# teasgen/speech_separation

Hardware: NVIDIA B200
Metric: dptn_av_separated_audio_seconds_per_second (higher is better)
Workload: dtype f16

## Files before the change

include/vatss.h:

```cpp
#ifndef VATSS_H_
#define VATSS_H_

#include <stddef.h>
#include <stdint.h>

#ifdef __cplusplus
extern "C" {
#endif

#define VATSS_ABI_VERSION 1

#define VATSS_KIND_DPTN_AV 0
#define VATSS_KIND_DPTN_WAV 1
#define VATSS_KIND_DPTN_MASK 2
#define VATSS_KIND_DPRNN 3

#define VATSS_ENGINE_AUTO 0
#define VATSS_ENGINE_GENERIC 1
#define VATSS_ENGINE_TENSOR 2
#define VATSS_ENGINE_TENSOR_F16RES 3

typedef struct vatss_model_desc {
  int32_t kind;
  int32_t N;
// ... 80 lines not shown
                    double* summary_out, double* scratch, void* stream);

int vatss_pit_sisdr(const float* s1p, const float* s2p, const float* s1, const float* s2, const float* mix, int B,
                    int T, int zero_mean, double* rows_out, double* summary_out, double* scratch, void* stream);

size_t vatss_sdr_workspace_bytes(int B, int T, int filter_length);
int vatss_sdr(const float* s1p, const float* s2p, const float* s1, const float* s2, const float* mix, int B, int T,
              int filter_length, int zero_mean, double load_diag, double* rows_out, double* summary_out,
              void* workspace, size_t workspace_bytes, void* stream);

int vatss_pit_sisnr_backward(const float* s1p, const float* s2p, const float* s1, const float* s2, int B, int T,
                             const double* scratch, const double* summary, const float* grad_out, float* grad_s1p,
                             float* grad_s2p, void* stream);

int vatss_tc_gemm(int epi, const void* A16, long long lda, const void* W16, const float* bias, const float* res,
                  long long ldr, const float* ln_w, const float* ln_b, float* out32, long long ldo32, void* out16,
                  long long ldo16, int act16, const float* prelu_a, long long M, int NOUT, int K, void* stream);

int vatss_tc_gemm_ln16(const void* A16, long long lda, const void* W16, const float* bias, const void* res16,
                       long long ldr16, const float* ln_w, const float* ln_b, float* out32, long long ldo32,
                       void* out16, long long ldo16, int act16, const float* prelu_a, long long M, int NOUT, int K,
                       void* stream);

int vatss_tc_lstm(const void* x16, const void* x16lo ,
                  const float* const* lstm_params ,
                  void* out16, int mode, int B, int S, int C, int N, int ndir, int act, void* wpack,
                  float* bias_pack, void* stream);

int vatss_tc_attention(const void* qkv16, void* out16, int mode, int B, int S, int C, int N, int heads, int force_simt,
                       void* stream);

int vatss_generic_gemm(const float* A, long long lda, const float* W, const float* bias, const float* bias2,
                       const float* R, long long ldr, float* out, long long ldc, long long M, int NOUT, int K, int act,
                       const float* prelu_a, void* stream);
int vatss_generic_layernorm(const float* in, const float* res, const float* w, const float* b, float* out,
                            long long rows, int N, int mode, void* stream);
int vatss_generic_attention(const float* qkv, float* out, int mode, int B, int S, int C, int N, int heads,
                            void* stream);
int vatss_generic_lstm(const float* pre, const float* whh_f, const float* whh_r, float* out, int mode, int B, int S,
                       int C, int H, int ndir, void* stream);

int vatss_tc_tail(const vatss_model_desc* d, const float* const* params, int n_params, const void* packed,
                  const void* x16, const float* enc, int B, int T, float* s1_pred, float* s2_pred,
                  void* workspace, size_t workspace_bytes, void* stream);

int vatss_longform_windows(int T, int W, int H);
int vatss_window_cut(const float* mix, const float* emb1, const float* emb2, int R, int T, int Tv, int E, int W, int H,
                     int spf, int first, int count, float* mix_out, float* emb1_out, float* emb2_out, void* stream);
size_t vatss_window_stitch_scratch_bytes(int R, int n);
int vatss_window_stitch(const float* y1, const float* y2, int R, int T, int W, int H, float* s1, float* s2,
                        uint8_t* swaps_out, double* corr_out, void* scratch, size_t scratch_bytes, void* stream);

size_t vatss_stoi_workspace_bytes(int B, int T, int fs);
int vatss_stoi(const float* s1p, const float* s2p, const float* s1, const float* s2, int B, int T, int fs, int extended,
               double* rows_out, int* kept_out, double* summary_out, void* workspace, size_t workspace_bytes,
               void* stream);

#define VATSS_STAGE_COUNT 9
unsigned long long vatss_launch_count(void);
void vatss_debug_lstm_trace(void* dev_buffer);
void vatss_debug_cta_limit(int ctas);
void vatss_debug_lstm_pingpong(int on);
void vatss_debug_lstm_groups(int groups);
void vatss_debug_tail_staged(int on);
void vatss_debug_gemm_l2_order(int on);
void vatss_debug_attention_version(int v);
int vatss_profile_begin(void);
int vatss_profile_end(float* ms_per_stage, int* launches_per_stage, int n_stages);

#define VATSS_LIP_NCONV 25
#define VATSS_LIP_PSLOTS 6
#define VATSS_LIP_ENGINE_F32 0
#define VATSS_LIP_ENGINE_TENSOR 1
void vatss_debug_lipreader(int flags);
void vatss_debug_lipreader_kernel(int version);
void vatss_debug_lipreader_trace(void* dev_buffer);
#define VATSS_LIP_NSTAGES 26
void vatss_debug_lipreader_capture(void* const* stages, int n);
size_t vatss_lipreader_packed_bytes(void);
size_t vatss_lipreader_workspace_bytes(int B, int T, int Hc, int Wc);
int vatss_lipreader_pack_weights(const float* const* params, int n_params, int relu_type, void* packed,
                                 size_t packed_bytes, void* stream);
int vatss_lipreader_forward(const void* packed, size_t packed_bytes, int relu_type, const float* video, int B, int T,
                            int Hin, int Win, int y0, int x0, int Hc, int Wc, float pre_scale, float pre_shift,
                            float* out, void* workspace, size_t workspace_bytes, int engine, void* stream);

#ifdef __cplusplus
}
#endif
// ... 2 lines not shown
```

speech_separation_b200/_lib.py:

```python
import ctypes
import os

_HERE = os.path.dirname(os.path.abspath(__file__))
LIB_PATH = os.environ.get("VATSS_LIB_OVERRIDE") or os.path.join(_HERE, "libvatss_b200.so")

KIND = {"dptn_av": 0, "dptn_wav": 1, "dptn_mask": 2, "dprnn": 3}
ENGINE = {"auto": 0, "generic": 1, "tensor": 2, "tensor-f16res": 3}

P_GLOBAL = [
    "encoder.weight", "decoder.weight", "visual_compression.weight", "visual_compression.bias", "gate",
    "video_ln.weight", "video_ln.bias", "dprnn.speakers_separation.0.weight",
    "dprnn.speakers_separation.1.weight", "dprnn.speakers_separation.1.bias",
    "HEAD_W", "HEAD_B", "dprnn.output_gate.0.weight", "dprnn.output_gate.0.bias",
]
S_DPTN = [
    "mha.in_proj_weight", "mha.in_proj_bias", "mha.out_proj.weight", "mha.out_proj.bias", "ln1.weight", "ln1.bias",
    "rnn.weight_ih_l0", "rnn.weight_hh_l0", "rnn.bias_ih_l0", "rnn.bias_hh_l0",
    "rnn.weight_ih_l0_reverse", "rnn.weight_hh_l0_reverse", "rnn.bias_ih_l0_reverse", "rnn.bias_hh_l0_reverse",
    "ffn.1.weight", "ffn.1.bias", "ln2.weight", "ln2.bias",
]
S_DPRNN = [
    None, None, None, None, None, None,
    "rnn.weight_ih_l0", "rnn.weight_hh_l0", "rnn.bias_ih_l0", "rnn.bias_hh_l0",
    "rnn.weight_ih_l0_reverse", "rnn.weight_hh_l0_reverse", "rnn.bias_ih_l0_reverse", "rnn.bias_hh_l0_reverse",
# ... 16 lines not shown
    "vatss_pack_weights": (ctypes.c_int, [ctypes.POINTER(ModelDesc), ctypes.POINTER(ctypes.c_void_p), ctypes.c_int,
                                          ctypes.c_void_p, ctypes.c_size_t, ctypes.c_void_p]),
    "vatss_forward": (ctypes.c_int, [ctypes.POINTER(ModelDesc), ctypes.POINTER(ctypes.c_void_p), ctypes.c_int,
                                     ctypes.c_void_p, ctypes.c_void_p, ctypes.c_void_p, ctypes.c_void_p,
                                     ctypes.c_int, ctypes.c_int, ctypes.c_int, ctypes.c_void_p, ctypes.c_void_p,
                                     ctypes.c_void_p, ctypes.c_size_t, ctypes.c_void_p]),
    "vatss_segment": (ctypes.c_int, [ctypes.c_void_p] + [ctypes.c_int] * 5 + [ctypes.c_void_p, ctypes.c_void_p]),
    "vatss_overlap_add": (ctypes.c_int, [ctypes.c_void_p] + [ctypes.c_int] * 5 + [ctypes.c_void_p, ctypes.c_void_p]),
    "vatss_encoder": (ctypes.c_int, [ctypes.POINTER(ModelDesc), ctypes.POINTER(ctypes.c_void_p), ctypes.c_void_p,
                                     ctypes.c_void_p, ctypes.c_void_p, ctypes.c_int, ctypes.c_int, ctypes.c_int,
                                     ctypes.c_void_p, ctypes.c_void_p, ctypes.c_void_p, ctypes.c_void_p]),
    "vatss_decoder": (ctypes.c_int, [ctypes.POINTER(ModelDesc), ctypes.c_void_p, ctypes.c_void_p, ctypes.c_int,
                                     ctypes.c_int, ctypes.c_void_p, ctypes.c_void_p, ctypes.c_void_p]),
    "vatss_tc_gemm": (ctypes.c_int, [ctypes.c_int, ctypes.c_void_p, ctypes.c_longlong, ctypes.c_void_p, ctypes.c_void_p,
                                     ctypes.c_void_p, ctypes.c_longlong, ctypes.c_void_p, ctypes.c_void_p,
                                     ctypes.c_void_p, ctypes.c_longlong, ctypes.c_void_p, ctypes.c_longlong,
                                     ctypes.c_int, ctypes.c_void_p, ctypes.c_longlong, ctypes.c_int, ctypes.c_int,
                                     ctypes.c_void_p]),
    "vatss_tc_gemm_ln16": (ctypes.c_int, [ctypes.c_void_p, ctypes.c_longlong, ctypes.c_void_p, ctypes.c_void_p,
                                          ctypes.c_void_p, ctypes.c_longlong, ctypes.c_void_p, ctypes.c_void_p,
                                          ctypes.c_void_p, ctypes.c_longlong, ctypes.c_void_p, ctypes.c_longlong,
                                          ctypes.c_int, ctypes.c_void_p, ctypes.c_longlong, ctypes.c_int, ctypes.c_int,
                                          ctypes.c_void_p]),
    "vatss_tc_lstm": (ctypes.c_int, [ctypes.c_void_p, ctypes.c_void_p, ctypes.POINTER(ctypes.c_void_p), ctypes.c_void_p] +
                      [ctypes.c_int] * 7 + [ctypes.c_void_p, ctypes.c_void_p, ctypes.c_void_p]),
    "vatss_tc_attention": (ctypes.c_int, [ctypes.c_void_p, ctypes.c_void_p] + [ctypes.c_int] * 7 + [ctypes.c_void_p]),
    "vatss_generic_gemm": (ctypes.c_int, [ctypes.c_void_p, ctypes.c_longlong] + [ctypes.c_void_p] * 4 +
                           [ctypes.c_longlong, ctypes.c_void_p, ctypes.c_longlong, ctypes.c_longlong, ctypes.c_int,
                            ctypes.c_int, ctypes.c_int, ctypes.c_void_p, ctypes.c_void_p]),
    "vatss_generic_layernorm": (ctypes.c_int, [ctypes.c_void_p] * 5 + [ctypes.c_longlong, ctypes.c_int, ctypes.c_int,
                                                                       ctypes.c_void_p]),
    "vatss_generic_attention": (ctypes.c_int, [ctypes.c_void_p, ctypes.c_void_p] + [ctypes.c_int] * 6 +
                                [ctypes.c_void_p]),
    "vatss_generic_lstm": (ctypes.c_int, [ctypes.c_void_p] * 4 + [ctypes.c_int] * 6 + [ctypes.c_void_p]),
    "vatss_tc_tail": (ctypes.c_int,[ctypes.POINTER(ModelDesc), ctypes.POINTER(ctypes.c_void_p), ctypes.c_int,
                                     ctypes.c_void_p, ctypes.c_void_p, ctypes.c_void_p, ctypes.c_int, ctypes.c_int,
                                     ctypes.c_void_p, ctypes.c_void_p, ctypes.c_void_p, ctypes.c_size_t,
                                     ctypes.c_void_p]),
    "vatss_launch_count": (ctypes.c_ulonglong, []),
    "vatss_engine_fallback_reason": (ctypes.c_char_p, [ctypes.POINTER(ModelDesc)]),
    "vatss_debug_lstm_trace": (None, [ctypes.c_void_p]),
    "vatss_debug_cta_limit": (None, [ctypes.c_int]),
    "vatss_debug_lstm_pingpong": (None, [ctypes.c_int]),
    "vatss_debug_lstm_groups": (None, [ctypes.c_int]),
    "vatss_debug_tail_staged": (None, [ctypes.c_int]),
    "vatss_debug_gemm_l2_order": (None, [ctypes.c_int]),
    "vatss_debug_attention_version": (None, [ctypes.c_int]),
    "vatss_profile_begin": (ctypes.c_int, []),
    "vatss_profile_end": (ctypes.c_int, [ctypes.POINTER(ctypes.c_float), ctypes.POINTER(ctypes.c_int), ctypes.c_int]),
    "vatss_sisnr_chunks": (ctypes.c_int, [ctypes.c_int]),
    "vatss_pit_sisnr": (ctypes.c_int, [ctypes.c_void_p] * 5 + [ctypes.c_int, ctypes.c_int] + [ctypes.c_void_p] * 5),
    "vatss_pit_sisdr": (ctypes.c_int, [ctypes.c_void_p] * 5 + [ctypes.c_int] * 3 + [ctypes.c_void_p] * 4),
    "vatss_sdr_workspace_bytes": (ctypes.c_size_t, [ctypes.c_int] * 3),
    "vatss_sdr": (ctypes.c_int, [ctypes.c_void_p] * 5 + [ctypes.c_int] * 4 + [ctypes.c_double] + [ctypes.c_void_p] * 3 +
                  [ctypes.c_size_t, ctypes.c_void_p]),
    "vatss_pit_sisnr_backward": (ctypes.c_int, [ctypes.c_void_p] * 4 + [ctypes.c_int, ctypes.c_int] + [ctypes.c_void_p] * 6),
    "vatss_longform_windows": (ctypes.c_int, [ctypes.c_int] * 3),
    "vatss_window_cut": (ctypes.c_int, [ctypes.c_void_p] * 3 + [ctypes.c_int] * 9 + [ctypes.c_void_p] * 4),
    "vatss_window_stitch_scratch_bytes": (ctypes.c_size_t, [ctypes.c_int, ctypes.c_int]),
    "vatss_window_stitch": (ctypes.c_int, [ctypes.c_void_p, ctypes.c_void_p] + [ctypes.c_int] * 4 +
                            [ctypes.c_void_p] * 5 + [ctypes.c_size_t, ctypes.c_void_p]),
    "vatss_stoi_workspace_bytes": (ctypes.c_size_t, [ctypes.c_int] * 3),
    "vatss_stoi": (ctypes.c_int, [ctypes.c_void_p] * 4 + [ctypes.c_int] * 4 + [ctypes.c_void_p] * 4 +
                   [ctypes.c_size_t, ctypes.c_void_p]),
    "vatss_debug_lipreader": (None, [ctypes.c_int]),
    "vatss_debug_lipreader_kernel": (None, [ctypes.c_int]),
    "vatss_debug_lipreader_trace": (None, [ctypes.c_void_p]),
    "vatss_debug_lipreader_capture": (None, [ctypes.POINTER(ctypes.c_void_p), ctypes.c_int]),
    "vatss_lipreader_packed_bytes": (ctypes.c_size_t, []),
    "vatss_lipreader_workspace_bytes": (ctypes.c_size_t, [ctypes.c_int] * 4),
# ... 76 lines not shown
```

speech_separation_b200/csrc/api.cu:

```cuda
#include <stdarg.h>
#include <string.h>

#include <atomic>
#include <mutex>
#include <string>
#include <vector>

#include "common.cuh"
#include "tensor_engine.cuh"
#include "tc_kernels.cuh"
#include "lipreader.cuh"

namespace vatss {

static thread_local std::string g_err;

void set_error(const char* fmt, ...) {
  char buf[1024];
  va_list ap;
  va_start(ap, fmt);
  vsnprintf(buf, sizeof(buf), fmt, ap);
  va_end(ap);
  g_err = buf;
}
// ... 346 lines not shown
  VATSS_CHECK_ARG(B > 0 && T >= d->K, "decoder: bad shape");
  const int L = (T - d->K) / stride_of(d) + 1;
  return launch_decoder(u, dec_w, B, L, d->N, d->K, T, proj_scratch, wav, (cudaStream_t)stream);
}

int vatss_tc_gemm(int epi, const void* A16, long long lda, const void* W16, const float* bias, const float* res,
                  long long ldr, const float* ln_w, const float* ln_b, float* out32, long long ldo32, void* out16,
                  long long ldo16, int act16, const float* prelu_a, long long M, int NOUT, int K, void* stream) {
  VATSS_CHECK_ARG(A16 && W16 && M >= 0, "tc_gemm: NULL operand");
  return launch_tc_gemm(epi, (const __half*)A16, lda, (const __half*)W16, bias, res, ldr, ln_w, ln_b, out32, ldo32,
                        (__half*)out16, ldo16, act16, prelu_a, M, NOUT, K, (cudaStream_t)stream);
}

int vatss_tc_gemm_ln16(const void* A16, long long lda, const void* W16, const float* bias, const void* res16,
                       long long ldr16, const float* ln_w, const float* ln_b, float* out32, long long ldo32,
                       void* out16, long long ldo16, int act16, const float* prelu_a, long long M, int NOUT, int K,
                       void* stream) {
  VATSS_CHECK_ARG(A16 && W16 && res16 && M >= 0, "tc_gemm_ln16: NULL operand");
  return launch_tc_gemm(TC_EPI_LN, (const __half*)A16, lda, (const __half*)W16, bias, nullptr, 0, ln_w, ln_b, out32,
                        ldo32, (__half*)out16, ldo16, act16, prelu_a, M, NOUT, K, (cudaStream_t)stream, nullptr, 0,
                        (const __half*)res16, ldr16);
}

int vatss_tc_lstm(const void* x16, const void* x16lo, const float* const* lp, void* out16, int mode, int B, int S, int C,
                  int N, int ndir, int act, void* wpack, float* bias_pack, void* stream) {
  VATSS_CHECK_ARG(x16 && lp && out16 && wpack && bias_pack, "tc_lstm: NULL pointer");
  VATSS_CHECK_ARG(ndir == 1 || ndir == 2, "tc_lstm: ndir must be 1 or 2");
  cudaStream_t st = (cudaStream_t)stream;
  for (int dir = 0; dir < ndir; ++dir) {
    int rc = launch_pack_lstm(lp[4 * dir + 0], lp[4 * dir + 1], lp[4 * dir + 2], lp[4 * dir + 3], N, dir,
                              x16lo != nullptr, (__half*)wpack, bias_pack, st);
    if (rc) return rc;
  }
  return launch_tc_lstm((const __half*)x16, (const __half*)x16lo, (const __half*)wpack, bias_pack, (__half*)out16, mode,
                        B, S, C, N, ndir,
                        act, st);
}

int vatss_tc_attention(const void* qkv16, void* out16, int mode, int B, int S, int C, int N, int heads, int force_simt,
                       void* stream) {
  VATSS_CHECK_ARG(qkv16 && out16 && heads > 0, "tc_attention: bad argument");
  const SeqMap map = mode == 0 ? intra_map(B, S, C) : inter_map(B, S, C);
  return launch_attention_f16((const __half*)qkv16, (__half*)out16, map, mode, B, S, C, N, heads, force_simt,
                              (cudaStream_t)stream);
}

// ... 30 lines not shown

int vatss_tc_tail(const vatss_model_desc* d, const float* const* params, int n_params, const void* packed,
                  const void* x16, const float* enc, int B, int T, float* s1_pred, float* s2_pred, void* workspace,
                  size_t workspace_bytes, void* stream) {
  if (check_desc(d)) return -1;
  VATSS_CHECK_ARG(params != nullptr && n_params == n_params_of(d), "parameter table has %d entries, expected %d",
                  n_params, n_params_of(d));
  VATSS_CHECK_ARG(tensor_engine_selected(d), "tc_tail: the model does not run on the TENSOR engine");
  VATSS_CHECK_ARG(packed && x16 && enc && s1_pred && s2_pred && workspace, "tc_tail: NULL pointer");
  Geometry g;
  if (geometry(d, B, T, 0, &g)) return -1;
  const size_t need = vatss_workspace_bytes(d, B, T, 0);
  VATSS_CHECK_ARG(workspace_bytes >= need, "workspace too small: %zu bytes given, %zu needed", workspace_bytes, need);
  return tensor_engine_tail(d, params, packed, (const __half*)x16, enc, g.B, g.T, 0, g.L, g.S, s1_pred, s2_pred,
                            workspace, (cudaStream_t)stream);
}

void vatss_debug_lstm_trace(void* dev_buffer) { vatss::g_lstm_trace = (long long*)dev_buffer; }
void vatss_debug_cta_limit(int ctas) { vatss::g_cta_limit = ctas; }
void vatss_debug_lstm_pingpong(int on) { vatss::g_lstm_pingpong = on; }
void vatss_debug_lstm_groups(int groups) { vatss::g_lstm_groups = groups; }
void vatss_debug_tail_staged(int on) { vatss::g_tail_staged = on; }
void vatss_debug_gemm_l2_order(int on) { vatss::g_gemm_l2_order = on; }
void vatss_debug_attention_version(int v) { vatss::g_attention_version = v == 1 ? 1 : 3; }

unsigned long long vatss_launch_count(void) { return g_launches.load(); }

int vatss_profile_begin(void) {
  std::lock_guard<std::mutex> lk(g_prof_mu);
  for (auto& r : g_prof) { cudaEventDestroy(r.a); cudaEventDestroy(r.b); }
  g_prof.clear();
  for (int i = 0; i < ST_COUNT; ++i) g_open[i] = -1;
  g_prof_on = true;
  return 0;
}

int vatss_profile_end(float* ms_per_stage, int* launches_per_stage, int n_stages) {
  std::lock_guard<std::mutex> lk(g_prof_mu);
  g_prof_on = false;
  VATSS_CHECK_ARG(ms_per_stage && launches_per_stage && n_stages >= ST_COUNT, "profile_end: need %d slots", ST_COUNT);
  for (int i = 0; i < n_stages; ++i) { ms_per_stage[i] = 0.f; launches_per_stage[i] = 0; }
  int rc = 0;
  for (auto& r : g_prof) {
    float ms = 0.f;
    if (cudaEventSynchronize(r.b) != cudaSuccess || cudaEventElapsedTime(&ms, r.a, r.b) != cudaSuccess) rc = -2;
    ms_per_stage[r.stage] += ms;
// ... 124 lines not shown
```

speech_separation_b200/csrc/tc_gemm.cu:

```cuda
#include "common.cuh"
#include "ptx.cuh"
#include "tc_kernels.cuh"

namespace vatss {

using namespace ptx;

typedef CUresult (*PFN_encodeTiled)(CUtensorMap*, CUtensorMapDataType, cuuint32_t, void*, const cuuint64_t*,
                                    const cuuint64_t*, const cuuint32_t*, const cuuint32_t*, CUtensorMapInterleave,
                                    CUtensorMapSwizzle, CUtensorMapL2promotion, CUtensorMapFloatOOBfill);

static PFN_encodeTiled get_encode() {
  static PFN_encodeTiled fn = nullptr;
  if (!fn) {
    void* p = nullptr;
    cudaDriverEntryPointQueryResult q;
    if (cudaGetDriverEntryPoint("cuTensorMapEncodeTiled", &p, cudaEnableDefault, &q) == cudaSuccess &&
        q == cudaDriverEntryPointSuccess)
      fn = reinterpret_cast<PFN_encodeTiled>(p);
  }
  return fn;
}

static int make_tmap_any(CUtensorMap* out, CUtensorMapDataType dt, const void* base, int rank, const uint64_t* dims,
// ... 571 lines not shown
  }
#define TCG_CASE(N_, K_, E_) \
  if (NOUT == N_ && KDIM == K_ && epi == E_) return tc_gemm_launch<N_, K_, E_>(A, lda, W, a, st);
  TCG_CASE(384, 128, TC_EPI_F16)
  TCG_CASE(128, 128, TC_EPI_LN)
  TCG_CASE(128, 256, TC_EPI_LN)
  TCG_CASE(128, 256, TC_EPI_LN_POST)
  TCG_CASE(128, 128, TC_EPI_LN_POST)
  TCG_CASE(256, 128, TC_EPI_F32)
  TCG_CASE(128, 128, TC_EPI_F32)
  TCG_CASE(192, 64, TC_EPI_F16)
  TCG_CASE(64, 64, TC_EPI_LN)
  TCG_CASE(64, 256, TC_EPI_LN)
  TCG_CASE(64, 128, TC_EPI_LN)
  TCG_CASE(64, 256, TC_EPI_LN_POST)
  TCG_CASE(64, 128, TC_EPI_LN_POST)
  TCG_CASE(128, 64, TC_EPI_F32)
  TCG_CASE(64, 64, TC_EPI_F32)
#undef TCG_CASE
  set_error("tc_gemm: no tensor-core instantiation for NOUT=%d K=%d epilogue=%d", NOUT, KDIM, epi);
  return -1;
}

}
```

speech_separation_b200/csrc/tc_kernels.cuh:

```cuda
#pragma once
#include <cuda_fp16.h>
#include <cuda_runtime.h>

#include "common.cuh"

namespace vatss {

enum { TC_EPI_F16 = 0, TC_EPI_F32 = 1, TC_EPI_LN = 2, TC_EPI_LN_POST = 3 };

int num_sms();
int grid_cap();
extern int g_cta_limit;
extern int g_lstm_pingpong;
extern int g_lstm_groups;
extern int g_tail_staged;
extern int g_gemm_l2_order;
extern long long* g_lstm_trace;

int launch_tc_gemm(int epi, const __half* A, long long lda, const __half* W, const float* bias, const float* res,
                   long long ldr, const float* ln_w, const float* ln_b, float* out32, long long ldo32, __half* out16,
                   long long ldo16, int act16, const float* prelu_a, long long M, int NOUT, int KDIM, cudaStream_t st,
                   __half* out16lo = nullptr, int wsplit = 0, const __half* res16 = nullptr, long long ldr16 = 0,
                   int reverse = 0, const __half* res16lo = nullptr);

int launch_tc_lstm(const __half* x16, const __half* x16lo, const __half* Wpack, const float* bias_pack, __half* out16,
                   int mode, int B, int S, int C, int NFEAT, int ndir, int act, cudaStream_t st);
int launch_pack_lstm(const float* Wih, const float* Whh, const float* bih, const float* bhh, int N, int dir,
                     int precise, __half* Wpack, float* bias_pack, cudaStream_t st);

int launch_attention_f16(const __half* qkv, __half* out, SeqMap map, int mode, int B, int S, int C, int N, int heads,
                         int force_simt, cudaStream_t st);

int launch_attention_v3(const __half* qkv, __half* out, SeqMap map, int mode, int B, int S, int C, int N, int heads,
                        cudaStream_t st);
extern int g_attention_version;

}
```

speech_separation_b200/csrc/tensor_engine.cu:

```cuda
#include "tensor_engine.cuh"

#include "tc_kernels.cuh"

#include <cstdlib>

namespace vatss {

int g_gemm_l2_order = -1;
int g_x16split = -1;
static bool x16split_enabled() {
  if (g_x16split < 0) {
    const char* e = getenv("VATSS_X16SPLIT");
    g_x16split = e ? atoi(e) : 1;
  }
  return g_x16split != 0;
}

namespace {

inline const float* sub_param(const float* const* params, int blk, int path, int slot) {
  return params[VATSS_P_GLOBAL_COUNT + (2 * blk + path) * VATSS_S_COUNT + slot];
}

struct Bump {
  char* base;
  size_t off = 0;
  explicit Bump(void* p) : base(reinterpret_cast<char*>(p)) {}
  template <typename T>
  T* take(size_t count) {
    T* r = reinterpret_cast<T*>(base + off);
    off += ((count * sizeof(T) + 1023) / 1024) * 1024;
    return r;
  }
};

struct SubPacked {
  __half* win;
  float* bin;
// ... 160 lines not shown
  if (d->kind == VATSS_KIND_DPTN_MASK) {
    if ((rc = to_half(params[VATSS_P_HGATE_W], p.wgate, N, N, 0, 1.f, st))) return rc;
  } else if ((rc = launch_fold_head(params[VATSS_P_HEAD_W], params[VATSS_P_HEAD_B], params[VATSS_P_DECODER_W], N, d->K,
                                    p.wfold, p.wdT, p.cfold, st)) ||
             (rc = launch_fold_spk(p.wfold, params[VATSS_P_SPK_W], params[VATSS_P_SPK_B], N, d->K, p.w2, p.c2, st))) {
    return rc;
  }
  return 0;
}

int tensor_engine_forward(const vatss_model_desc* d, const float* const* params, const void* packed,
                          const float* mix, const float* emb1, const float* emb2, int B, int T, int Tv, int L,
                          int S, float* s1_pred, float* s2_pred, void* workspace, cudaStream_t st) {
  Packed p;
  carve_packed(d, const_cast<void*>(packed), &p);
  Work w;
  carve_work(d, B, Tv, L, S, workspace, &w);
  const int N = d->N, H = d->H, C = d->C;
  const long long tok = (long long)B * S * C;
  const bool dprnn = d->kind == VATSS_KIND_DPRNN, av = d->kind == VATSS_KIND_DPTN_AV;
  const bool f16res = d->engine == VATSS_ENGINE_TENSOR_F16RES && !dprnn && d->kind != VATSS_KIND_DPTN_MASK;
  const bool y16res = d->kind != VATSS_KIND_DPTN_MASK;
  const bool x16split = !dprnn && d->kind != VATSS_KIND_DPTN_MASK && !f16res && x16split_enabled();
  int rc;
  {
    StageScope sc(ST_FRONTEND, st);
    if (av) {
      VATSS_CHECK_ARG(emb1 && emb2 && Tv > 0, "DPTN-AV needs both lip-embedding streams (Tv=%d)", Tv);
      if ((rc = launch_visual_compress(emb1, emb2, params[VATSS_P_VIS_W], params[VATSS_P_VIS_B], B, d->E, Tv, N, w.vis,
                                       st)))
        return rc;
    }
    if ((rc = launch_encoder(mix, params[VATSS_P_ENCODER_W], av ? w.vis : nullptr, params[VATSS_P_GATE],
                             params[VATSS_P_VLN_W], params[VATSS_P_VLN_B], B, T, Tv, N, d->K, L, S, C, d->P, w.enc32,
                             (f16res || x16split) ? nullptr : w.xa32, w.xa16, st, (dprnn || x16split) ? w.xa16lo : nullptr)))
      return rc;
  }
  for (int blk = 0; blk < d->num_blocks; ++blk)
    for (int path = 0; path < 2; ++path) {
      const int ndir = (path == 0 || d->bidir) ? 2 : 1;
      const SubPacked& s = p.sub[2 * blk + path];
      auto sp = [&](int slot) { return sub_param(params, blk, path, slot); };
      const SeqMap map = path == 0 ? intra_map(B, S, C) : inter_map(B, S, C);
      const bool last = (blk == d->num_blocks - 1) && path == 1;
      if (dprnn) {
        {
          StageScope sc(ST_LSTM_RECURRENT, st);
          if ((rc = launch_tc_lstm(w.xa16, w.xa16lo, s.wlstm, s.blstm, w.rnn16, path, B, S, C, N, ndir, 0, st))) return rc;
        }
        StageScope sc(ST_FFN_LN, st);
        if ((rc = launch_tc_gemm(TC_EPI_LN_POST, w.rnn16, ndir * H, s.wffn, sp(VATSS_S_FFN_B), w.xa32, N,
                                 sp(VATSS_S_LN2_W), sp(VATSS_S_LN2_B), w.xb32, N, w.xb16, N, last ? 2 : 0,
                                 params[VATSS_P_PRELU], tok, N, ndir * H, st, last ? nullptr : w.xb16lo, 1)))
          return rc;
        float* t32 = w.xa32; w.xa32 = w.xb32; w.xb32 = t32;
        __half* t16 = w.xa16; w.xa16 = w.xb16; w.xb16 = t16;
        t16 = w.xa16lo; w.xa16lo = w.xb16lo; w.xb16lo = t16;
      } else {
        {
          StageScope sc(ST_QKV, st);
          if ((rc = launch_tc_gemm(TC_EPI_F16, w.xa16, N, s.win, s.bin, nullptr, 0, nullptr, nullptr, nullptr, 0,
                                   w.qkv16, 3 * N, 0, nullptr, tok, 3 * N, N, st, nullptr, 0, nullptr, 0, g_gemm_l2_order)))
            return rc;
        }
        {
          StageScope sc(ST_ATTENTION, st);
          if ((rc = launch_attention_f16(w.qkv16, w.att16, map, path, B, S, C, N, d->heads, 0, st))) return rc;
        }
        {
          StageScope sc(ST_OUTPROJ_LN, st);
          if ((rc = launch_tc_gemm(TC_EPI_LN, w.att16, N, s.wout, sp(VATSS_S_OUTPROJ_B),
                                   (f16res || x16split) ? nullptr : w.xa32, N, sp(VATSS_S_LN1_W), sp(VATSS_S_LN1_B),
                                   y16res ? nullptr : w.xb32, N, w.xb16, N, 0, nullptr, tok, N, N, st, nullptr, 0,
                                   (f16res || x16split) ? w.xa16 : nullptr, N, g_gemm_l2_order,
                                   x16split ? w.xa16lo : nullptr)))
            return rc;
        }
        {
          StageScope sc(ST_LSTM_RECURRENT, st);
          if ((rc = launch_tc_lstm(w.xb16, nullptr, s.wlstm, s.blstm, w.rnn16, path, B, S, C, N, ndir, 1, st))) return rc;
        }
        StageScope sc(ST_FFN_LN, st);
        if ((rc = launch_tc_gemm(TC_EPI_LN, w.rnn16, ndir * H, s.wffn, sp(VATSS_S_FFN_B), y16res ? nullptr : w.xb32, N,
                                 sp(VATSS_S_LN2_W), sp(VATSS_S_LN2_B), (f16res || x16split || last) ? nullptr : w.xa32, N,
                                 w.xa16, N, last ? 2 : 0, params[VATSS_P_PRELU], tok, N, ndir * H, st,
                                 (x16split && !last) ? w.xa16lo : nullptr, 0, y16res ? w.xb16 : nullptr, N)))
          return rc;
      }
    }
  return tensor_engine_tail(d, params, packed, w.xa16, w.enc32, B, T, Tv, L, S, s1_pred, s2_pred, workspace, st);
}

int tensor_engine_tail(const vatss_model_desc* d, const float* const* params, const void* packed, const __half* x16,
                       const float* enc32, int B, int T, int Tv, int L, int S, float* s1_pred, float* s2_pred,
                       void* workspace, cudaStream_t st) {
  Packed p;
  carve_packed(d, const_cast<void*>(packed), &p);
  Work w;
  carve_work(d, B, Tv, L, S, workspace, &w);
  const int N = d->N, C = d->C;
  const long long tok = (long long)B * S * C, fr = (long long)B * L;
  int rc;
  StageScope sc(ST_TAIL, st);
  float* preds[2] = {s1_pred, s2_pred};
  if (d->kind != VATSS_KIND_DPTN_MASK) {
    rc = launch_tail_fused(x16, enc32, p.w2, p.c2, p.wdT, p.cfold, B, S, C, d->P, L, N, d->K, w.proj, st);
// ... 32 lines not shown
```

Baseline: 4354.

## Fuse FFN+LayerNorm GEMM with next sublayer's QKV projection in one kernel

Adds a clustered tcgen05 kernel that computes the FFN GEMM with residual add and LayerNorm, writes the normalized hi/lo f16 activations, and then reuses that tile from shared memory as the A operand for the following sublayer's QKV projection. The tensor engine calls it by default (env-controlled) for every non-last sublayer and skips the separate QKV GEMM. This removes one launch per sublayer and avoids re-reading the activation from global memory for QKV. In exchange it keeps both weight sets resident in shared memory and adds a more complex warp-specialized pipeline with cross-CTA barriers.

```diff
diff --git a/include/vatss.h b/include/vatss.h
--- a/include/vatss.h
+++ b/include/vatss.h
@@ -126,6 +126,10 @@
                        void* out16, long long ldo16, int act16, const float* prelu_a, long long M, int NOUT, int K,
                        void* stream);
 
+int vatss_tc_ffn_qkv(const void* rnn16, int KF, const void* Wffn16, const float* bffn, const void* y16,
+                     const float* ln_w, const float* ln_b, void* x16, void* x16lo, const void* Wqkv16,
+                     const float* bqkv, void* qkv16, long long M, int N, int fused, void* stream);
+
 int vatss_tc_lstm(const void* x16, const void* x16lo ,
                   const float* const* lstm_params ,
                   void* out16, int mode, int B, int S, int C, int N, int ndir, int act, void* wpack,
@@ -169,6 +173,7 @@
 void vatss_debug_tail_staged(int on);
 void vatss_debug_gemm_l2_order(int on);
 void vatss_debug_attention_version(int v);
+void vatss_debug_ffn_qkv_fused(int on);
 int vatss_profile_begin(void);
 int vatss_profile_end(float* ms_per_stage, int* launches_per_stage, int n_stages);
 
diff --git a/speech_separation_b200/_lib.py b/speech_separation_b200/_lib.py
--- a/speech_separation_b200/_lib.py
+++ b/speech_separation_b200/_lib.py
@@ -62,6 +62,8 @@
                                           ctypes.c_void_p, ctypes.c_longlong, ctypes.c_void_p, ctypes.c_longlong,
                                           ctypes.c_int, ctypes.c_void_p, ctypes.c_longlong, ctypes.c_int, ctypes.c_int,
                                           ctypes.c_void_p]),
+    "vatss_tc_ffn_qkv": (ctypes.c_int, [ctypes.c_void_p, ctypes.c_int] + [ctypes.c_void_p] * 10 +
+                         [ctypes.c_longlong, ctypes.c_int, ctypes.c_int, ctypes.c_void_p]),
     "vatss_tc_lstm": (ctypes.c_int, [ctypes.c_void_p, ctypes.c_void_p, ctypes.POINTER(ctypes.c_void_p), ctypes.c_void_p] +
                       [ctypes.c_int] * 7 + [ctypes.c_void_p, ctypes.c_void_p, ctypes.c_void_p]),
     "vatss_tc_attention": (ctypes.c_int, [ctypes.c_void_p, ctypes.c_void_p] + [ctypes.c_int] * 7 + [ctypes.c_void_p]),
@@ -86,6 +88,7 @@
     "vatss_debug_tail_staged": (None, [ctypes.c_int]),
     "vatss_debug_gemm_l2_order": (None, [ctypes.c_int]),
     "vatss_debug_attention_version": (None, [ctypes.c_int]),
+    "vatss_debug_ffn_qkv_fused": (None, [ctypes.c_int]),
     "vatss_profile_begin": (ctypes.c_int, []),
     "vatss_profile_end": (ctypes.c_int, [ctypes.POINTER(ctypes.c_float), ctypes.POINTER(ctypes.c_int), ctypes.c_int]),
     "vatss_sisnr_chunks": (ctypes.c_int, [ctypes.c_int]),
diff --git a/speech_separation_b200/csrc/api.cu b/speech_separation_b200/csrc/api.cu
--- a/speech_separation_b200/csrc/api.cu
+++ b/speech_separation_b200/csrc/api.cu
@@ -392,6 +392,22 @@
                         (const __half*)res16, ldr16);
 }
 
+int vatss_tc_ffn_qkv(const void* rnn16, int KF, const void* Wffn16, const float* bffn, const void* y16,
+                     const float* ln_w, const float* ln_b, void* x16, void* x16lo, const void* Wqkv16,
+                     const float* bqkv, void* qkv16, long long M, int N, int fused, void* stream) {
+  VATSS_CHECK_ARG(M >= 0, "tc_ffn_qkv: negative row count");
+  cudaStream_t st = (cudaStream_t)stream;
+  if (fused)
+    return launch_tc_ffn_qkv((const __half*)rnn16, KF, (const __half*)Wffn16, bffn, (const __half*)y16, ln_w, ln_b,
+                             (__half*)x16, (__half*)x16lo, (const __half*)Wqkv16, bqkv, (__half*)qkv16, M, N, st);
+  int rc = launch_tc_gemm(TC_EPI_LN, (const __half*)rnn16, KF, (const __half*)Wffn16, bffn, nullptr, N, ln_w, ln_b,
+                          nullptr, N, (__half*)x16, N, 0, nullptr, M, N, KF, st, (__half*)x16lo, 0,
+                          (const __half*)y16, N);
+  if (rc) return rc;
+  return launch_tc_gemm(TC_EPI_F16, (const __half*)x16, N, (const __half*)Wqkv16, bqkv, nullptr, 0, nullptr, nullptr,
+                        nullptr, 0, (__half*)qkv16, 3 * N, 0, nullptr, M, 3 * N, N, st);
+}
+
 int vatss_tc_lstm(const void* x16, const void* x16lo, const float* const* lp, void* out16, int mode, int B, int S, int C,
                   int N, int ndir, int act, void* wpack, float* bias_pack, void* stream) {
   VATSS_CHECK_ARG(x16 && lp && out16 && wpack && bias_pack, "tc_lstm: NULL pointer");
@@ -468,6 +484,7 @@
 void vatss_debug_lstm_groups(int groups) { vatss::g_lstm_groups = groups; }
 void vatss_debug_tail_staged(int on) { vatss::g_tail_staged = on; }
 void vatss_debug_gemm_l2_order(int on) { vatss::g_gemm_l2_order = on; }
+void vatss_debug_ffn_qkv_fused(int on) { vatss::g_ffn_qkv_fused = on; }
 void vatss_debug_attention_version(int v) { vatss::g_attention_version = v == 1 ? 1 : 3; }
 
 unsigned long long vatss_launch_count(void) { return g_launches.load(); }
diff --git a/speech_separation_b200/csrc/tc_gemm.cu b/speech_separation_b200/csrc/tc_gemm.cu
--- a/speech_separation_b200/csrc/tc_gemm.cu
+++ b/speech_separation_b200/csrc/tc_gemm.cu
@@ -617,4 +617,398 @@
   return -1;
 }
 
-}
+template <int N, int KF>
+struct FfnQkvSmem {
+  static constexpr int KBF = KF / 64;
+  static constexpr int KBQ = N / 64;
+  static constexpr int WROW = (N / 2) * 128;
+  static constexpr int OFF_WF = 0;
+  static constexpr int OFF_WQ = OFF_WF + KBF * WROW;
+  static constexpr int OFF_A = OFF_WQ + 3 * KBQ * WROW;
+  static constexpr int OFF_Y = OFF_A + KBF * 16384;
+  static constexpr int OFF_PAR = OFF_Y + KBQ * 16384;
+  static constexpr int OFF_BAR = OFF_PAR + 6 * N * 4;
+  static constexpr int OFF_XCH = OFF_BAR + 256;
+  static constexpr int OFF_STAGE = OFF_XCH + 2048;
+  static constexpr int EPW = 8;
+  static constexpr int THREADS = 64 + 32 * EPW;
+  static constexpr int TOTAL = OFF_STAGE + EPW * 32 * STG_LD * 4 + 1024;
+  static constexpr int TMEM_COLS = 4 * N <= 256 ? 256 : 512;
+  static_assert(4 * N <= 512 && N % 64 == 0 && KF % 64 == 0, "shape");
+};
+
+struct FfnQkvArgs {
+  long long M;
+  int num_pairs;
+  const float* bffn;
+  const float* ln_w;
+  const float* ln_b;
+  const float* bqkv;
+  __half* x16;
+  __half* x16lo;
+  __half* qkv16;
+};
+
+template <int N, int KF>
+__global__ void __cluster_dims__(2, 1, 1) __launch_bounds__(FfnQkvSmem<N, KF>::THREADS, 1)
+k_tc_ffn_qkv(const __grid_constant__ CUtensorMap tmapA, const __grid_constant__ CUtensorMap tmapY,
+             const __grid_constant__ CUtensorMap tmapWf, const __grid_constant__ CUtensorMap tmapWq, FfnQkvArgs p) {
+  using L = FfnQkvSmem<N, KF>;
+  extern __shared__ unsigned char smem_raw[];
+  const uint32_t base = (smem_u32(smem_raw) + 1023u) & ~1023u;
+  unsigned char* gen = smem_raw + (base - smem_u32(smem_raw));
+  const uint32_t sWf = base + L::OFF_WF, sWq = base + L::OFF_WQ, sA = base + L::OFF_A, sY = base + L::OFF_Y;
+  float* sPar = reinterpret_cast<float*>(gen + L::OFF_PAR);
+  const uint32_t bars = base + L::OFF_BAR;
+  const uint32_t bar_w = bars;
+  const uint32_t bar_afull = bars + 8;
+  const uint32_t bar_aempty = bars + 16;
+  const uint32_t bar_yfull = bars + 24;
+  const uint32_t bar_yempty = bars + 32;
+  const uint32_t bar_ffull = bars + 40;
+  const uint32_t bar_fempty = bars + 56;
+  const uint32_t bar_xfull = bars + 72;
+  const uint32_t bar_qfull = bars + 80;
+  const uint32_t bar_qempty = bars + 96;
+  const uint32_t tmem_slot = bars + 128;
+
+  const int warp = threadIdx.x >> 5, lane = threadIdx.x & 31;
+  const uint32_t rank = cluster_ctarank();
+  const bool leader = rank == 0;
+  const int cluster = blockIdx.x >> 1, nclusters = gridDim.x >> 1;
+
+  if (threadIdx.x == 0) {
+    mbar_init(bar_w, 1);
+    mbar_init(bar_afull, 1);
+    mbar_init(bar_aempty, 1);
+    mbar_init(bar_yfull, 1);
+    mbar_init(bar_yempty, 1);
+    mbar_init(bar_xfull, 2 * L::EPW);
+    for (int s = 0; s < 2; ++s) {
+      mbar_init(bar_ffull + 8 * s, 1);
+      mbar_init(bar_fempty + 8 * s, 2 * L::EPW);
+      mbar_init(bar_qfull + 8 * s, 1);
+      mbar_init(bar_qempty + 8 * s, 2 * L::EPW);
+    }
+    fence_mbar_init();
+    prefetch_tmap(&tmapA);
+    prefetch_tmap(&tmapY);
+    prefetch_tmap(&tmapWf);
+    prefetch_tmap(&tmapWq);
+  }
+  for (int i = threadIdx.x; i < N; i += blockDim.x) {
+    sPar[i] = p.bffn[i];
+    sPar[N + i] = p.ln_w[i];
+    sPar[2 * N + i] = p.ln_b[i];
+  }
+  for (int i = threadIdx.x; i < 3 * N; i += blockDim.x) sPar[3 * N + i] = p.bqkv[i];
+  if (warp == 1) {
+    tmem_alloc<2>(tmem_slot, L::TMEM_COLS);
+    tmem_relinquish<2>();
+  }
+  tc_fence_before();
+  __syncthreads();
+  cluster_sync();
+  tc_fence_after();
+  const uint32_t tmem = *reinterpret_cast<volatile uint32_t*>(gen + L::OFF_BAR + 128);
+
+  if (threadIdx.x == 0) {
+    mbar_expect_tx(bar_w, (L::KBF + 3 * L::KBQ) * L::WROW);
+    for (int kb = 0; kb < L::KBF; ++kb) tma_load_2d(sWf + kb * L::WROW, &tmapWf, bar_w, kb * 64, (int)rank * (N / 2));
+    for (int ch = 0; ch < 3; ++ch)
+      for (int kb = 0; kb < L::KBQ; ++kb)
+        tma_load_2d(sWq + (ch * L::KBQ + kb) * L::WROW, &tmapWq, bar_w, kb * 64, ch * N + (int)rank * (N / 2));
+  }
+  mbar_wait(bar_w, 0);
+  cluster_sync();
+
+  if (warp == 0) {
+    if (lane == 0) {
+      uint32_t afull_leader;
+      asm volatile("mapa.shared::cluster.u32 %0, %1, 0;" : "=r"(afull_leader) : "r"(bar_afull));
+      int i = 0;
+      for (int pt = cluster; pt < p.num_pairs; pt += nclusters, ++i) {
+        const int row0 = pt * 256 + (int)rank * 128;
+        mbar_wait(bar_aempty, (i & 1) ^ 1);
+        if (leader) mbar_expect_tx(bar_afull, 2 * L::KBF * 16384);
+        for (int kb = 0; kb < L::KBF; ++kb) tma_load_2d_cg2(sA + kb * 16384, &tmapA, afull_leader, kb * 64, row0);
+        mbar_wait(bar_yempty, (i & 1) ^ 1);
+        mbar_expect_tx(bar_yfull, L::KBQ * 16384);
+        for (int cb = 0; cb < L::KBQ; ++cb) tma_load_2d(sY + cb * 16384, &tmapY, bar_yfull, cb * 64, row0);
+      }
+    }
+    __syncwarp();
+  } else if (warp == 1) {
+    if (leader && lane == 0) {
+      constexpr uint32_t IDESC = idesc_f16(256, N, 0);
+      int i = 0;
+      for (int pt = cluster; pt < p.num_pairs; pt += nclusters, ++i) {
+        const int fs = i & 1;
+        mbar_wait(bar_afull, i & 1);
+        mbar_wait(bar_fempty + 8 * fs, ((i >> 1) & 1) ^ 1);
+        tc_fence_after();
+#pragma unroll
+        for (int k16 = 0; k16 < KF / 16; ++k16) {
+          const int kb = k16 >> 2, kk = k16 & 3;
+          const uint64_t a = smem_desc_sw128_kmajor(sA + kb * 16384) + (uint64_t)(kk * 2);
+          const uint64_t b = smem_desc_sw128_kmajor(sWf + kb * L::WROW) + (uint64_t)(kk * 2);
+          umma_f16<2>(tmem + fs * N, a, b, IDESC, k16 > 0 ? 1u : 0u);
+        }
+        umma_commit_cg2(bar_aempty, 3);
+        umma_commit_cg2(bar_ffull + 8 * fs, 3);
+        mbar_wait(bar_xfull, i & 1);
+        tc_fence_after();
+#pragma unroll
+        for (int ch = 0; ch < 3; ++ch) {
+          const int j = i * 3 + ch, qs = j & 1;
+          mbar_wait(bar_qempty + 8 * qs, ((j >> 1) & 1) ^ 1);
+          tc_fence_after();
+#pragma unroll
+          for (int k16 = 0; k16 < N / 16; ++k16) {
+            const int kb = k16 >> 2, kk = k16 & 3;
+            const uint64_t a = smem_desc_sw128_kmajor(sY + kb * 16384) + (uint64_t)(kk * 2);
+            const uint64_t b = smem_desc_sw128_kmajor(sWq + (ch * L::KBQ + kb) * L::WROW) + (uint64_t)(kk * 2);
+            umma_f16<2>(tmem + 2 * N + qs * N, a, b, IDESC, k16 > 0 ? 1u : 0u);
+          }
+          if (ch == 2) umma_commit_cg2(bar_yempty, 3);
+          umma_commit_cg2(bar_qfull + 8 * qs, 3);
+        }
+      }
+    }
+    __syncwarp();
+  } else {
+    const int q = warp & 3, half = (warp - 2) >> 2;
+    constexpr int NC = N / 2;
+    const int cbase = half * NC;
+    const int rr = q * 32 + lane;
+    const float* sBias = sPar;
+    const float* sLw = sPar + N;
+    const float* sLb = sPar + 2 * N;
+    const float* sBq = sPar + 3 * N;
+    float* xch = reinterpret_cast<float*>(gen + L::OFF_XCH);
+    float* stage = reinterpret_cast<float*>(gen + L::OFF_STAGE) + (warp - 2) * 32 * STG_LD;
+    uint32_t fempty_leader[2], qempty_leader[2], xfull_leader;
+    for (int s = 0; s < 2; ++s) {
+      asm volatile("mapa.shared::cluster.u32 %0, %1, 0;" : "=r"(fempty_leader[s]) : "r"(bar_fempty + 8 * s));
+      asm volatile("mapa.shared::cluster.u32 %0, %1, 0;" : "=r"(qempty_leader[s]) : "r"(bar_qempty + 8 * s));
+    }
+    asm volatile("mapa.shared::cluster.u32 %0, %1, 0;" : "=r"(xfull_leader) : "r"(bar_xfull));
+    auto arrive_leader = [&](uint32_t bar) {
+      __syncwarp();
+      if (lane == 0) asm volatile("mbarrier.arrive.shared::cluster.b64 _, [%0];" ::"r"(bar) : "memory");
+    };
+    int i = 0;
+    for (int pt = cluster; pt < p.num_pairs; pt += nclusters, ++i) {
+      const long long row0 = (long long)pt * 256 + rank * 128 + q * 32;
+      const long long left = p.M - row0;
+      const int rows_valid = left >= 32 ? 32 : (left > 0 ? (int)left : 0);
+      const int fs = i & 1;
+      float v[NC];
+      mbar_wait(bar_yfull, i & 1);
+      mbar_wait(bar_ffull + 8 * fs, (i >> 1) & 1);
+      tc_fence_after();
+#pragma unroll
+      for (int c0 = 0; c0 < NC; c0 += 32) {
+        uint32_t r[32];
+        tmem_ld_32x32b_x32(tmem + ((uint32_t)(q * 32) << 16) + fs * N + cbase + c0, r);
+        tmem_ld_wait();
+#pragma unroll
+        for (int j = 0; j < 32; ++j) v[c0 + j] = __uint_as_float(r[j]) + sBias[cbase + c0 + j];
+        const int col = cbase + c0;
+#pragma unroll
+        for (int c = 0; c < 4; ++c) {
+          const uint4 x = *reinterpret_cast<const uint4*>(gen + L::OFF_Y + (col / 64) * 16384 +
+                                                          sw128_offset((uint32_t)rr, (uint32_t)((col % 64) / 8 + c)));
+          add_half2(v[c0 + 8 * c], v[c0 + 8 * c + 1], x.x);
+          add_half2(v[c0 + 8 * c + 2], v[c0 + 8 * c + 3], x.y);
+          add_half2(v[c0 + 8 * c + 4], v[c0 + 8 * c + 5], x.z);
+          add_half2(v[c0 + 8 * c + 6], v[c0 + 8 * c + 7], x.w);
+        }
+      }
+      tc_fence_before();
+      arrive_leader(fs ? fempty_leader[1] : fempty_leader[0]);
+      float sum = 0.f;
+#pragma unroll
+      for (int j = 0; j < NC; ++j) sum += v[j];
+      xch[half * 256 + rr] = sum;
+      asm volatile("bar.sync %0, 64;" ::"r"(1 + q) : "memory");
+      sum += xch[(half ^ 1) * 256 + rr];
+      const float mean = sum * (1.f / N);
+      float sq = 0.f;
+#pragma unroll
+      for (int j = 0; j < NC; ++j) {
+        const float d = v[j] - mean;
+        sq = fmaf(d, d, sq);
+      }
+      xch[half * 256 + 128 + rr] = sq;
+      asm volatile("bar.sync %0, 64;" ::"r"(1 + q) : "memory");
+      sq += xch[(half ^ 1) * 256 + 128 + rr];
+      const float rstd = rsqrtf(sq * (1.f / N) + 1e-5f);
+#pragma unroll
+      for (int j = 0; j < NC; ++j) v[j] = (v[j] - mean) * rstd * sLw[cbase + j] + sLb[cbase + j];
+#pragma unroll
+      for (int c0 = 0; c0 < NC; c0 += 32) {
+        const int col = cbase + c0;
+#pragma unroll
+        for (int c = 0; c < 4; ++c) {
+          uint32_t pk[4];
+#pragma unroll
+          for (int e = 0; e < 4; ++e) {
+            const __half2 h = __floats2half2_rn(v[c0 + 8 * c + 2 * e], v[c0 + 8 * c + 2 * e + 1]);
+            pk[e] = *reinterpret_cast<const uint32_t*>(&h);
+          }
+          *reinterpret_cast<uint4*>(gen + L::OFF_Y + (col / 64) * 16384 +
+                                    sw128_offset((uint32_t)rr, (uint32_t)((col % 64) / 8 + c))) =
+              make_uint4(pk[0], pk[1], pk[2], pk[3]);
+        }
+      }
+      fence_proxy_async();
+      arrive_leader(xfull_leader);
+#pragma unroll
+      for (int c0 = 0; c0 < NC; c0 += 32) {
+        const int col = cbase + c0;
+        uint32_t pk[16];
+#pragma unroll
+        for (int j = 0; j < 16; ++j) {
+          const __half2 h = __floats2half2_rn(v[c0 + 2 * j], v[c0 + 2 * j + 1]);
+          pk[j] = *reinterpret_cast<const uint32_t*>(&h);
+        }
+        staged_store_f16(p.x16 + row0 * N + col, N, rows_valid, stage, lane, pk);
+#pragma unroll
+        for (int j = 0; j < 16; ++j) {
+          const float2 hf = __half22float2(*reinterpret_cast<const __half2*>(&pk[j]));
+          const __half2 lo = __floats2half2_rn(v[c0 + 2 * j] - hf.x, v[c0 + 2 * j + 1] - hf.y);
+          pk[j] = *reinterpret_cast<const uint32_t*>(&lo);
+        }
+        staged_store_f16(p.x16lo + row0 * N + col, N, rows_valid, stage, lane, pk);
+      }
+      constexpr int PPC = N / 64;
+      uint32_t* st = reinterpret_cast<uint32_t*>(stage);
+      const int wsw = (lane >> 1) & 3;
+#pragma unroll 1
+      for (int ch = 0; ch < 3; ++ch) {
+        const int j = i * 3 + ch, qs = j & 1;
+        mbar_wait(bar_qfull + 8 * qs, (j >> 1) & 1);
+        tc_fence_after();
+        uint32_t r[PPC][32];
+#pragma unroll
+        for (int pc = 0; pc < PPC; ++pc)
+          tmem_ld_32x32b_x32(tmem + ((uint32_t)(q * 32) << 16) + 2 * N + qs * N + half * 32 + 64 * pc, r[pc]);
+        tmem_ld_wait();
+        tc_fence_before();
+        arrive_leader(qs ? qempty_leader[1] : qempty_leader[0]);
+        const int c0 = ch * N + half * 32;
+#pragma unroll
+        for (int pc = 0; pc < PPC; ++pc)
+#pragma unroll
+          for (int jj = 0; jj < 4; ++jj) {
+            uint32_t a[4];
+#pragma unroll
+            for (int e = 0; e < 4; ++e) {
+              const int c = 8 * jj + 2 * e;
+              const __half2 h = __floats2half2_rn(__uint_as_float(r[pc][c]) + sBq[c0 + 64 * pc + c],
+                                                  __uint_as_float(r[pc][c + 1]) + sBq[c0 + 64 * pc + c + 1]);
+              a[e] = *reinterpret_cast<const uint32_t*>(&h);
+            }
+            *reinterpret_cast<uint4*>(st + pc * 512 + lane * 16 + ((jj ^ wsw) << 2)) = make_uint4(a[0], a[1], a[2], a[3]);
+          }
+        __syncwarp();
+        __half* g = p.qkv16 + row0 * (3 * N) + c0;
+#pragma unroll
+        for (int k = 0; k < 4; ++k) {
+          const int r8 = k * 8 + (lane >> 2), c = lane & 3;
+#pragma unroll
+          for (int pc = 0; pc < PPC; ++pc) {
+            const uint4 x = *reinterpret_cast<const uint4*>(st + pc * 512 + r8 * 16 + ((c ^ ((r8 >> 1) & 3)) << 2));
+            if (r8 < rows_valid) *reinterpret_cast<uint4*>(g + (long long)r8 * (3 * N) + 64 * pc + c * 8) = x;
+          }
+        }
+        __syncwarp();
+      }
+    }
+  }
+  tc_fence_before();
+  __syncthreads();
+  cluster_sync();
+  if (warp == 1) tmem_dealloc<2>(tmem, L::TMEM_COLS);
+}
+
+template <int N, int KF>
+static int ffn_qkv_launch(const __half* rnn16, const __half* Wffn, const __half* y16, const __half* Wqkv,
+                          const FfnQkvArgs& a, cudaStream_t st) {
+  using L = FfnQkvSmem<N, KF>;
+  static_assert(L::TOTAL <= 227 * 1024, "shared memory budget");
+  auto kern = k_tc_ffn_qkv<N, KF>;
+  CUtensorMap tmA, tmY, tmWf, tmWq;
+  {
+    const uint64_t dims[2] = {(uint64_t)KF, (uint64_t)a.M};
+    const uint64_t str[1] = {(uint64_t)KF * 2};
+    const uint32_t box[2] = {64, 128};
+    if (make_tmap_f16(&tmA, rnn16, 2, dims, str, box)) return -1;
+  }
+  {
+    const uint64_t dims[2] = {(uint64_t)N, (uint64_t)a.M};
+    const uint64_t str[1] = {(uint64_t)N * 2};
+    const uint32_t box[2] = {64, 128};
+    if (make_tmap_f16(&tmY, y16, 2, dims, str, box)) return -1;
+  }
+  {
+    const uint64_t dims[2] = {(uint64_t)KF, (uint64_t)N};
+    const uint64_t str[1] = {(uint64_t)KF * 2};
+    const uint32_t box[2] = {64, N / 2};
+    if (make_tmap_f16(&tmWf, Wffn, 2, dims, str, box)) return -1;
+  }
+  {
+    const uint64_t dims[2] = {(uint64_t)N, (uint64_t)(3 * N)};
+    const uint64_t str[1] = {(uint64_t)N * 2};
+    const uint32_t box[2] = {64, N / 2};
+    if (make_tmap_f16(&tmWq, Wqkv, 2, dims, str, box)) return -1;
+  }
+  static int max_clusters[64] = {0};
+  int dev = 0;
+  cudaGetDevice(&dev);
+  static PerDeviceOnce configured;
+  if (configured.first()) {
+    VATSS_CUDA_OK(cudaFuncSetAttribute(kern, cudaFuncAttributeMaxDynamicSharedMemorySize, L::TOTAL));
+    cudaLaunchConfig_t cfg = {};
+    cfg.gridDim = dim3(2 * (num_sms() / 2), 1, 1);
+    cfg.blockDim = dim3(L::THREADS, 1, 1);
+    cfg.dynamicSmemBytes = L::TOTAL;
+    int n = 0;
+    if (cudaOccupancyMaxActiveClusters(&n, kern, &cfg) != cudaSuccess) {
+      (void)cudaGetLastError();
+      n = num_sms() / 2;
+    }
+    max_clusters[dev & 63] = n > 0 ? n : 1;
+  }
+  int clusters = max_clusters[dev & 63];
+  if (clusters > grid_cap() / 2) clusters = grid_cap() / 2 > 0 ? grid_cap() / 2 : 1;
+  if (clusters > a.num_pairs) clusters = a.num_pairs;
+  kern<<<2 * clusters, L::THREADS, L::TOTAL, st>>>(tmA, tmY, tmWf, tmWq, a);
+  VATSS_LAUNCH_OK();
+  return 0;
+}
+
+int launch_tc_ffn_qkv(const __half* rnn16, int KF, const __half* Wffn, const float* bffn, const __half* y16,
+                      const float* ln_w, const float* ln_b, __half* x16, __half* x16lo, const __half* Wqkv,
+                      const float* bqkv, __half* qkv16, long long M, int N, cudaStream_t st) {
+  if (M == 0) return 0;
+  VATSS_CHECK_ARG(rnn16 && Wffn && bffn && y16 && ln_w && ln_b && x16 && x16lo && Wqkv && bqkv && qkv16,
+                  "tc_ffn_qkv: NULL operand");
+  VATSS_CHECK_ARG(((uintptr_t)rnn16 & 15) == 0 && ((uintptr_t)y16 & 15) == 0 && ((uintptr_t)x16 & 15) == 0 &&
+                      ((uintptr_t)x16lo & 15) == 0 && ((uintptr_t)qkv16 & 15) == 0,
+                  "tc_ffn_qkv: activations must be 16-byte aligned");
+  FfnQkvArgs a;
+  a.M = M;
+  a.num_pairs = (int)((M + 255) / 256);
+  a.bffn = bffn; a.ln_w = ln_w; a.ln_b = ln_b; a.bqkv = bqkv;
+  a.x16 = x16; a.x16lo = x16lo; a.qkv16 = qkv16;
+  if (N == 128 && KF == 256) return ffn_qkv_launch<128, 256>(rnn16, Wffn, y16, Wqkv, a, st);
+  if (N == 128 && KF == 128) return ffn_qkv_launch<128, 128>(rnn16, Wffn, y16, Wqkv, a, st);
+  if (N == 64 && KF == 256) return ffn_qkv_launch<64, 256>(rnn16, Wffn, y16, Wqkv, a, st);
+  if (N == 64 && KF == 128) return ffn_qkv_launch<64, 128>(rnn16, Wffn, y16, Wqkv, a, st);
+  set_error("tc_ffn_qkv: no instantiation for N=%d KF=%d", N, KF);
+  return -1;
+}
+
+}
diff --git a/speech_separation_b200/csrc/tc_kernels.cuh b/speech_separation_b200/csrc/tc_kernels.cuh
--- a/speech_separation_b200/csrc/tc_kernels.cuh
+++ b/speech_separation_b200/csrc/tc_kernels.cuh
@@ -15,6 +15,7 @@
 extern int g_lstm_groups;
 extern int g_tail_staged;
 extern int g_gemm_l2_order;
+extern int g_ffn_qkv_fused;
 extern long long* g_lstm_trace;
 
 int launch_tc_gemm(int epi, const __half* A, long long lda, const __half* W, const float* bias, const float* res,
@@ -22,6 +23,10 @@
                    long long ldo16, int act16, const float* prelu_a, long long M, int NOUT, int KDIM, cudaStream_t st,
                    __half* out16lo = nullptr, int wsplit = 0, const __half* res16 = nullptr, long long ldr16 = 0,
                    int reverse = 0, const __half* res16lo = nullptr);
+
+int launch_tc_ffn_qkv(const __half* rnn16, int KF, const __half* Wffn, const float* bffn, const __half* y16,
+                      const float* ln_w, const float* ln_b, __half* x16, __half* x16lo, const __half* Wqkv,
+                      const float* bqkv, __half* qkv16, long long M, int N, cudaStream_t st);
 
 int launch_tc_lstm(const __half* x16, const __half* x16lo, const __half* Wpack, const float* bias_pack, __half* out16,
                    int mode, int B, int S, int C, int NFEAT, int ndir, int act, cudaStream_t st);
diff --git a/speech_separation_b200/csrc/tensor_engine.cu b/speech_separation_b200/csrc/tensor_engine.cu
--- a/speech_separation_b200/csrc/tensor_engine.cu
+++ b/speech_separation_b200/csrc/tensor_engine.cu
@@ -14,6 +14,14 @@
     g_x16split = e ? atoi(e) : 1;
   }
   return g_x16split != 0;
+}
+int g_ffn_qkv_fused = -1;
+static bool ffn_qkv_fused_enabled() {
+  if (g_ffn_qkv_fused < 0) {
+    const char* e = getenv("VATSS_FFN_QKV_FUSED");
+    g_ffn_qkv_fused = e ? atoi(e) : 1;
+  }
+  return g_ffn_qkv_fused != 0;
 }
 
 namespace {
@@ -220,6 +228,8 @@
   const bool f16res = d->engine == VATSS_ENGINE_TENSOR_F16RES && !dprnn && d->kind != VATSS_KIND_DPTN_MASK;
   const bool y16res = d->kind != VATSS_KIND_DPTN_MASK;
   const bool x16split = !dprnn && d->kind != VATSS_KIND_DPTN_MASK && !f16res && x16split_enabled();
+  const bool fuse_ffn_qkv = x16split && ffn_qkv_fused_enabled();
+  bool qkv_ready = false;
   int rc;
   {
     StageScope sc(ST_FRONTEND, st);
@@ -255,7 +265,7 @@
         __half* t16 = w.xa16; w.xa16 = w.xb16; w.xb16 = t16;
         t16 = w.xa16lo; w.xa16lo = w.xb16lo; w.xb16lo = t16;
       } else {
-        {
+        if (!qkv_ready) {
           StageScope sc(ST_QKV, st);
           if ((rc = launch_tc_gemm(TC_EPI_F16, w.xa16, N, s.win, s.bin, nullptr, 0, nullptr, nullptr, nullptr, 0,
                                    w.qkv16, 3 * N, 0, nullptr, tok, 3 * N, N, st, nullptr, 0, nullptr, 0, g_gemm_l2_order)))
@@ -279,7 +289,13 @@
           if ((rc = launch_tc_lstm(w.xb16, nullptr, s.wlstm, s.blstm, w.rnn16, path, B, S, C, N, ndir, 1, st))) return rc;
         }
         StageScope sc(ST_FFN_LN, st);
-        if ((rc = launch_tc_gemm(TC_EPI_LN, w.rnn16, ndir * H, s.wffn, sp(VATSS_S_FFN_B), y16res ? nullptr : w.xb32, N,
+        qkv_ready = fuse_ffn_qkv && !last;
+        if (qkv_ready) {
+          const SubPacked& nx = p.sub[2 * blk + path + 1];
+          if ((rc = launch_tc_ffn_qkv(w.rnn16, ndir * H, s.wffn, sp(VATSS_S_FFN_B), w.xb16, sp(VATSS_S_LN2_W),
+                                      sp(VATSS_S_LN2_B), w.xa16, w.xa16lo, nx.win, nx.bin, w.qkv16, tok, N, st)))
+            return rc;
+        } else if ((rc = launch_tc_gemm(TC_EPI_LN, w.rnn16, ndir * H, s.wffn, sp(VATSS_S_FFN_B), y16res ? nullptr : w.xb32, N,
                                  sp(VATSS_S_LN2_W), sp(VATSS_S_LN2_B), (f16res || x16split || last) ? nullptr : w.xa32, N,
                                  w.xa16, N, last ? 2 : 0, params[VATSS_P_PRELU], tok, N, ndir * H, st,
                                  (x16split && !last) ? w.xa16lo : nullptr, 0, y16res ? w.xb16 : nullptr, N)))
```

New measurement: 4426 (median of 6 runs). +1.6%, better.
